# IamJerryXu/Multimodal-Diagnosis-HAM-Spine

Measured on AMD Instinct MI355X. Metric: training images/sec, ResNet50+BERT-base 224px bs32, higher is better.
Workload: dtype bf16; 1 GPU; C2: ResNet50 + BERT-base(L=128) + cross-attention FusionModule + MLP head, 224x224, batch 32 per GPU, CE(label_smoothing=0.02), fused AdamW, train-mode BatchNorm and dropout; per_gpu_batch=32, global_batch=32, seq_len=128, params=134897991, parallelism=dp1

## Files before the change

include/hamspine.h:

```cpp
#ifndef HAMSPINE_H
#define HAMSPINE_H

#include <stdint.h>

#ifdef __cplusplus
extern "C" {
#endif

typedef int hs_status;
enum { HS_OK = 0, HS_ERR_ARG = 1, HS_ERR_HIP = 2, HS_ERR_UNSUPPORTED = 3 };
enum { HS_F32 = 0, HS_BF16 = 1 };

const char* hs_last_error(void);
int hs_version(void);
int hs_device_ok(void);


enum {
    HS_A_KC = 0,
    HS_A_RC = 1,
    HS_A_CONV = 2,
    HS_A_DGRAD = 3
};
enum {
// ... 519 lines not shown
    float* dword;
    float* dpos;
    float* dtype0;
    float* dgamma;
    float* dbeta;
    int32_t n_layers;
    hs_bert_layer_desc layers[HS_BERT_MAX_LAYERS];
    int32_t pack_rows;
} hs_bert_desc;
int32_t hs_bert_pack_rows_available(void);
hs_status hs_bert_query(const hs_bert_desc* d, int64_t* saved_bytes, int64_t* ws_bytes, int64_t* out_offset);
hs_status hs_bert_fwd(const hs_bert_desc* d, const int64_t* ids, const int64_t* mask, void* saved, int64_t saved_bytes,
                      void* ws, int64_t ws_bytes, void* stream);
hs_status hs_bert_bwd(const hs_bert_desc* d, const int64_t* ids, const int64_t* mask, const void* dy, void* saved,
                      int64_t saved_bytes, void* ws, int64_t ws_bytes, void* stream);

hs_status hs_linear_fwd(int32_t dtype, const void* x, int64_t M, int32_t ldx, const hs_linear* lin, const void* w_lp,
                        void* y, int32_t ldy, int32_t out_dtype, int32_t act, void* preact, const void* residual,
                        int32_t ldr, float dropout_p, uint64_t seed, void* stream);
hs_status hs_linear_bwd(int32_t dtype, const void* x, int64_t M, int32_t ldx, const hs_linear* lin, const void* w_lp,
                        const void* dy, int32_t ldy, void* dx, int32_t lddx, int32_t dx_dtype, int32_t mul_mode,
                        const void* mul_src, int32_t ldm, const void* dx_residual, void* ws, int64_t ws_bytes,
                        void* stream);
int64_t hs_linear_bwd_ws_bytes(int64_t M, int32_t in_f, int32_t out_f, int32_t dtype);

hs_status hs_tta_expand(const float* x, float* out, int64_t planes, int32_t H, int32_t W, const int32_t* ops, int32_t V,
                        void* stream);
hs_status hs_group_mean(const float* x, float* out, int32_t V, int64_t n, void* stream);
hs_status hs_repeat(int32_t elem_bytes, const void* x, void* out, int64_t n, int32_t V, void* stream);
hs_status hs_gradcam(int32_t dtype, const void* act, const void* grad, float* cam, int32_t B, int32_t C, int32_t HW,
// ... 35 lines not shown
```

multimodal-diagnosis-ham-spine_amd/hamspine/csrc/blocks.hip:

```cpp
#include <algorithm>
#include <atomic>
#include <mutex>
#include <unordered_map>
#include <vector>
#include "hs_internal.h"
#include "hs_switch.h"
#include "pw_stream.h"

namespace hs {

__global__ __launch_bounds__(256) void gather3_kernel(const float* __restrict__ a, const float* __restrict__ b,
                                                      const float* __restrict__ c, float* __restrict__ dst, int n) {
    const int i = blockIdx.x * 256 + threadIdx.x;
    if (i >= 3 * n) return;
    const int w = i / n, k = i - w * n;
    dst[i] = w == 0 ? a[k] : (w == 1 ? b[k] : c[k]);
}

static inline long long align_up(long long v, long long a) { return (v + a - 1) / a * a; }
static inline int esize(int dt) { return dt == HS_BF16 ? 2 : 4; }

struct Arena {
    char* base = nullptr;
    long long cap = 0, off = 0, peak = 0;
// ... 22 lines not shown
        saved.base = (char*)saved_base; saved.cap = saved_bytes;
        ws.base = (char*)ws_base; ws.cap = ws_bytes;
    }
    hipStream_t side = nullptr;
    bool side_used = false;
    bool defer_wgrad = false;
    GemmGroup *grp_pw = nullptr, *grp_conv = nullptr;
    bool group_nt = false;
    GemmGroup* grp_nt = nullptr;
    GemmGroup* tower_grp = nullptr;
    struct PendTr { const void* src; void* dst; int R, C; long long ld; unsigned char tok; };
    std::vector<PendTr> pend_tr;
    const int *pk_T = nullptr, *pk_cu = nullptr, *pk_row = nullptr, *pk_inv = nullptr;
    const int *pk_kc = nullptr, *pk_kcpos = nullptr, *pk_kcols = nullptr;
    bool kc_on = false;
};

static hipStream_t g_side_stream[16] = {};
static hipEvent_t g_events[16][64] = {};
static int g_event_next[16] = {};
static std::mutex g_side_mu;
static int side_setup(Run& r) {
    if (r.plan || !sw::overlap()) return HS_OK;
    int dev = 0;
    HS_CHECK_HIP(hipGetDevice(&dev));
    if (dev < 0 || dev >= 16) return HS_OK;
    std::lock_guard<std::mutex> lk(g_side_mu);
    if (!g_side_stream[dev]) HS_CHECK_HIP(hipStreamCreateWithFlags(&g_side_stream[dev], hipStreamNonBlocking));
    r.side = g_side_stream[dev];
    return HS_OK;
// ... 1242 lines not shown
    HS_PROPAGATE(linear_fwd_run(r, x, M, Hd, qkv_lin, L.wqkv, L.qkv, 3 * Hd, r.dt, HS_ACT_NONE, nullptr, nullptr, 0, 0.f, 0));
    hs_attn_desc a = bert_attn_desc(d, r.dt);
    const char* qkv = (const char*)L.qkv;
    HS_PROPAGATE(attention_fwd_run(r, a, qkv, qkv ? qkv + (long long)Hd * es : nullptr,
                                   qkv ? qkv + 2ll * Hd * es : nullptr, L.ctx));
    HS_PROPAGATE(linear_fwd_run(r, L.ctx, M, Hd, d.ao, L.wao, L.h1, Hd, r.dt, HS_ACT_NONE, nullptr, x, Hd, d.hidden_dropout,
                                d.seed * 8 + 2));
    CALL(r, ln_fwd(r.dt, L.h1, d.ln1.gamma, d.ln1.beta, L.x1, L.mean1, L.rstd1, M, Hd, d.ln_eps, r.s, r.pk_T));
    HS_PROPAGATE(linear_fwd_run(r, L.x1, M, Hd, d.inter_l, L.wi, L.g, I, r.dt, HS_ACT_GELU, L.u, nullptr, 0, 0.f, 0));
    HS_PROPAGATE(linear_fwd_run(r, L.g, M, I, d.out_l, L.wo, L.h2, Hd, r.dt, HS_ACT_NONE, nullptr, L.x1, Hd,
                                d.hidden_dropout, d.seed * 8 + 3));
    CALL(r, ln_fwd(r.dt, L.h2, d.ln2.gamma, d.ln2.beta, y, L.mean2, L.rstd2, M, Hd, d.ln_eps, r.s, r.pk_T));
    RUN_CHECK_ARENAS(r, "bert_layer_fwd");
    return HS_OK;
}
static int bert_layer_bwd_run(Run& r, const hs_bert_layer_desc& d, const void* x, const void* dy, void* dx) {
    BertLayout L;
    HS_PROPAGATE(bert_layout(r, d, L));
    const int Hd = d.hidden, I = d.inter;
    const long long M = (long long)d.B * d.L;
    const int es = esize(r.dt);
    hs_attn_desc a = bert_attn_desc(d, r.dt);
    void* dh2 = r.ws.alloc(M * Hd * es);
    void* dd2 = r.ws.alloc(M * Hd * es);
    void* dh1 = r.ws.alloc(M * Hd * es);
    void* dd1 = r.ws.alloc(M * Hd * es);
    void* du = r.ws.alloc(M * I * es);
    void* dx1 = r.ws.alloc(M * Hd * es);
    void* dctx = r.ws.alloc(M * Hd * es);
    void* dqkv = r.ws.alloc(M * 3 * Hd * es);
// ... 5 lines not shown
    const bool fuse_ln = sw::fused_ln_bwd();
    const void* g2 = d.hidden_dropout > 0.f ? dd2 : dh2;
    hs_linear out_l_w = d.out_l;
    if (fuse_ln) {
        CALL(r, ln_bwd_pre(r.dt, dy, L.h2, d.ln2.gamma, L.mean2, L.rstd2, dh2, d.ln2.dgamma ? d.ln2.dgamma : scratch,
                           d.ln2.dbeta ? d.ln2.dbeta : (scratch ? scratch + Hd : nullptr),
                           d.hidden_dropout > 0.f ? dd2 : nullptr, d.out_l.db, d.hidden_dropout, d.seed * 8 + 3,
                           ln_ws, ln_ws_bytes, M, Hd, r.s, r.pk_inv));
        out_l_w.db = nullptr;
    } else {
        CALLK(r, 128, ln_bwd(r.dt, dy, L.h2, d.ln2.gamma, L.mean2, L.rstd2, dh2, d.ln2.dgamma ? d.ln2.dgamma : scratch,
                             d.ln2.dbeta ? d.ln2.dbeta : (scratch ? scratch + Hd : nullptr), ln_ws, ln_ws_bytes, M, Hd, r.s, r.pk_inv));
        if (d.hidden_dropout > 0.f && r.pk_T) CALL(r, dropout_rows(r.dt, dh2, dd2, M, Hd, d.hidden_dropout, d.seed * 8 + 3, r.pk_T, r.pk_row, r.s));
        else if (d.hidden_dropout > 0.f) CALL(r, hs_dropout(r.dt, dh2, dd2, M * Hd, d.hidden_dropout, d.seed * 8 + 3, r.s));
    }
    const bool nt = r.dt == HS_BF16 && sw::wgrad_nt() && M % 8 == 0 && Hd % 8 == 0 && I % 8 == 0;
    HS_REQUIRE(!r.pk_T || nt, "bert_layer_bwd: packed rows need the transposed-operand weight gradients (bf16, HAMSPINE_WGRAD_NT on)");
    const long long big_tiles = (long long)ceil_div(3 * Hd, 256) * ceil_div(Hd, 128) + (long long)ceil_div(Hd, 256) * ceil_div(Hd, 128) +
                                (long long)ceil_div(I, 256) * ceil_div(Hd, 128) + (long long)ceil_div(Hd, 256) * ceil_div(I, 128);
    const bool grouped = nt && sw::grouped_bert_wgrad() && !sw::overlap() && big_tiles >= 128;
    char* tA = nt ? (char*)r.ws.alloc(M * (long long)std::max(3 * Hd, I) * 2) : nullptr;
    char* tA_ffn2 = grouped ? (char*)r.ws.alloc(M * (long long)Hd * 2) : tA;
    char* tA_ao = grouped ? (char*)r.ws.alloc(M * (long long)Hd * 2) : tA;
    char* tA_qkv = grouped ? (char*)r.ws.alloc(M * 3ll * Hd * 2) : tA;
    r.group_nt = grouped;
    if (grouped && !r.plan) {
        r.grp_nt = r.tower_grp ? r.tower_grp : gemm_group_open(r.s, (long long)(uintptr_t)d.q.w + 16);
        HS_REQUIRE(r.grp_nt != nullptr, "bert_layer_bwd: cannot set up the grouped weight-gradient launch");
    }
    r.kc_on = r.pk_T && r.pk_kcols && grouped && !r.plan && sw::bert_wgrad_chunks() && gemm_group_takes_k_cols();
    const int* const k_cols = r.kc_on ? r.pk_kcols : nullptr;
    char* tX_g = nt ? (char*)r.ws.alloc(M * (long long)I * 2) : nullptr;
    char* tX_x1 = nt ? (char*)r.ws.alloc(M * (long long)Hd * 2) : nullptr;
    char* tX_ctx = nt ? (char*)r.ws.alloc(M * (long long)Hd * 2) : nullptr;
    char* tX_x = nt ? (char*)r.ws.alloc(M * (long long)Hd * 2) : nullptr;
    auto bias_by_colsum = [&](const hs_linear& lin, const void* dy_rm, int ldy) -> int {
        hs_linear only_b = lin;
        only_b.dw = nullptr;
        return linear_wgrad_run(r, nullptr, M, 0, only_b, dy_rm, ldy);
    };
    auto wgrad = [&](const void* x_rm, const void* xT, int in_f, const hs_linear& lin, const void* dy_rm, int ldy, char* tAk) -> int {
        if (!nt || !lin.dw) {
            const bool keep = r.group_nt;
            r.group_nt = false;
            const int st = linear_wgrad_run(r, x_rm, M, in_f, lin, dy_rm, ldy);
            r.group_nt = keep;
            return st;
        }
        HS_PROPAGATE(transpose_run(r, dy_rm, tAk, M, lin.out_f, ldy, true, true));
        const bool fused_b = lin.db && (r.group_nt || hs_gemm_suggest_split(lin.out_f, in_f, (int)M, r.dt) <= 1) && sw::fused_bias_grad();
        HS_PROPAGATE(linear_wgrad_nt_run(r, xT, tAk, M, in_f, lin.out_f, lin.dw, lin.db, 0, nullptr, nullptr, k_cols));
        if (lin.db && !fused_b) HS_PROPAGATE(bias_by_colsum(lin, dy_rm, ldy));
        return HS_OK;
    };
    const bool dnt = r.dt == HS_BF16 && sw::dgrad_nt() && Hd % 8 == 0 && I % 8 == 0;
    char* wo_t = dnt ? (char*)r.ws.alloc((long long)Hd * I * 2) : nullptr;
    char* wi_t = dnt ? (char*)r.ws.alloc((long long)Hd * I * 2) : nullptr;
    char* wqkv_t = dnt ? (char*)r.ws.alloc(3ll * Hd * Hd * 2) : nullptr;
    {
        const void* src[7];
        void* dst[7];
        int32_t R[7], Cc[7];
        int64_t lds[7], ldd[7];
        unsigned char tok[7];
        int n = 0;
        auto add = [&](const void* s_, void* d_, long long rows, int cols, bool tokens = false) {
            src[n] = s_; dst[n] = d_; R[n] = (int32_t)rows; Cc[n] = cols; lds[n] = cols; ldd[n] = rows; tok[n] = tokens ? (r.kc_on ? 2 : 1) : 0;
            ++n;
        };
        if (nt) {
            add(L.g, tX_g, M, I, true);
            add(L.x1, tX_x1, M, Hd, true);
            add(L.ctx, tX_ctx, M, Hd, true);
            add(x, tX_x, M, Hd, true);
// ... 252 lines not shown
    const hs_conv_bn& cb = d.stem.cb;
    if (cb.dw || cb.dgamma || cb.dbeta) {
        r.saved.off = lo.lay_off[0];
        const long long wm = r.ws.mark();
        HS_PROPAGATE(stem_bwd_run(r, d.stem, r.saved.base ? r.saved.base + lo.y_off[0] : nullptr, dy));
        r.ws.release(wm);
    }
    return milestones_flush(r);
}

struct BertTowerLayout {
    long long ssum_off, stats_off;
    long long y_off[HS_BERT_MAX_LAYERS + 1], lay_off[HS_BERT_MAX_LAYERS + 1];
    long long act_bytes;
    long long map_off, out_off;
};
static void bert_pack_pointers(Run& r, const hs_bert_desc& d, const BertTowerLayout& lo) {
    const int* map = (const int*)(r.saved.base + lo.map_off);
    r.pk_T = map;
    r.pk_cu = map + 4;
    r.pk_row = r.pk_cu + (d.B + 1 + 3) / 4 * 4;
    r.pk_inv = r.pk_row + (long long)d.B * d.L;
    r.pk_kc = map + 1;
    r.pk_kcpos = r.pk_inv + (long long)d.B * d.L;
}
static int bert_check(const hs_bert_desc& d) {
    HS_REQUIRE(d.n_layers >= 0 && d.n_layers <= HS_BERT_MAX_LAYERS, "bert: n_layers %d out of range", d.n_layers);
    HS_REQUIRE(d.B > 0 && d.L > 0 && d.hidden > 0 && d.vocab > 0, "bert: bad dims");
    HS_REQUIRE(d.word && d.pos && d.type0 && d.gamma && d.beta, "bert: null embedding parameter");
    for (int i = 0; i < d.n_layers; ++i)
        HS_REQUIRE(d.layers[i].dtype == d.dtype && d.layers[i].B == d.B && d.layers[i].L == d.L && d.layers[i].hidden == d.hidden,
// ... 3 lines not shown
        for (int i = 0; i < d.n_layers; ++i) {
            const hs_bert_layer_desc& l = d.layers[i];
            HS_REQUIRE(l.heads > 0 && d.hidden == 64 * l.heads && l.inter % 8 == 0, "bert: pack_rows needs head dim 64 (layer %d)", i);
            const int wanted = (l.q.dw != nullptr) + (l.k.dw != nullptr) + (l.v.dw != nullptr);
            HS_REQUIRE(wanted == 0 || wanted == 3, "bert: pack_rows needs the q / k / v weight gradients of layer %d all wanted or all frozen", i);
        }
    }
    return HS_OK;
}
static hs_bert_layer_desc bert_layer_of(const hs_bert_desc& d, int i, const int64_t* mask) {
    hs_bert_layer_desc l = d.layers[i];
    l.attention_mask = mask;
    l.seed = d.seed + 16ull * (unsigned)(i + 1);
    return l;
}
static int bert_fwd_run(Run& r, const hs_bert_desc& d, const int64_t* ids, const int64_t* mask, BertTowerLayout& lo) {
    const long long M = (long long)d.B * d.L;
    const int es = esize(d.dtype);
    lo.act_bytes = M * d.hidden * es;
    lo.map_off = lo.out_off = 0;
    char* out_pad = nullptr;
    if (d.pack_rows) {
        HS_REQUIRE(r.plan || mask, "bert_fwd: pack_rows needs an attention mask");
        lo.map_off = r.saved.mark();
        int* map = (int*)r.saved.alloc(bert_row_map_bytes(d.B, d.L));
        lo.out_off = r.saved.mark();
        out_pad = (char*)r.saved.alloc(lo.act_bytes);
        if (!r.plan) {
            RUN_CHECK_ARENAS(r, "bert_fwd(row map)");
            HS_PROPAGATE(bert_row_map(mask, d.B, d.L, map, r.s));
            bert_pack_pointers(r, d, lo);
// ... 7 lines not shown
    char* x = (char*)r.saved.alloc(lo.act_bytes);
    lo.lay_off[0] = r.saved.mark();
    CALL(r, bert_embed_fwd_rows(d.dtype, ids, d.word, d.pos, d.type0, d.gamma, d.beta, ssum, x, stats, stats + M, M, d.L, d.hidden,
                                d.vocab, d.ln_eps, d.embed_dropout, d.seed, r.pk_T, r.pk_row, r.s));
    for (int i = 0; i < d.n_layers; ++i) {
        lo.y_off[i + 1] = r.saved.mark();
        char* y = (char*)r.saved.alloc(lo.act_bytes);
        lo.lay_off[i + 1] = r.saved.mark();
        const hs_bert_layer_desc l = bert_layer_of(d, i, mask);
        const long long wm = r.ws.mark();
        HS_PROPAGATE(bert_layer_fwd_run(r, l, x, y));
        r.ws.release(wm);
        x = y;
    }
    if (d.pack_rows) CALL(r, bert_unpack_rows(x, out_pad, M, (long long)d.hidden * es, r.pk_inv, r.s));
    return HS_OK;
}
static int bert_bwd_run(Run& r, const hs_bert_desc& d, const int64_t* ids, const int64_t* mask, const void* dy_in,
                        const BertTowerLayout& lo) {
    const long long M = (long long)d.B * d.L;
    const int Hd = d.hidden;
    char* dy_packed = d.pack_rows ? (char*)r.ws.alloc(lo.act_bytes) : nullptr;
    int* kcols = d.pack_rows ? (int*)r.ws.alloc(sizeof(int)) : nullptr;
    char* gbuf[2] = {(char*)r.ws.alloc(lo.act_bytes), (char*)r.ws.alloc(lo.act_bytes)};
    int cur = 0;
    const void* dy = dy_in;
    char* base = r.saved.base;
    if (d.pack_rows && !r.plan) {
        RUN_CHECK_ARENAS(r, "bert_bwd(row map)");
        bert_pack_pointers(r, d, lo);
        HS_PROPAGATE(bert_pack_rows(dy_in, dy_packed, M, (long long)Hd * esize(d.dtype), r.pk_T, r.pk_row, r.pk_kc + 1, kcols, r.s));
        r.pk_kcols = kcols;
        dy = dy_packed;
    }
// ... 1 lines not shown
    int pending = 0;
    long long wm = 0;
    const void* gps[8][16];
    struct HookGuard {
        explicit HookGuard(Run* rr) { gemm_group_set_immediate_hook([](void* c) -> int { return pending_transposes_flush(*(Run*)c); }, rr); }
        ~HookGuard() { gemm_group_set_immediate_hook(nullptr, nullptr); }
    } hook_guard(&r);
    for (int i = d.n_layers - 1; i >= 0; --i) {
        const hs_bert_layer_desc l = bert_layer_of(d, i, mask);
        char* dx = gbuf[cur];
        r.saved.off = lo.lay_off[i + 1];
        if (pending == 0) {
            wm = r.ws.mark();
            r.tower_grp = (span > 1 && !r.plan) ? gemm_group_open(r.s, (long long)(uintptr_t)l.q.w + 24) : nullptr;
        }
        HS_PROPAGATE(bert_layer_bwd_run(r, l, base ? base + lo.y_off[i] : nullptr, dy, dx));
        {
            const void* gp[16] = {l.q.dw, l.q.db, l.k.dw, l.k.db, l.v.dw, l.v.db, l.ao.dw, l.ao.db, l.ln1.dgamma, l.ln1.dbeta,
                                  l.inter_l.dw, l.inter_l.db, l.out_l.dw, l.out_l.db, l.ln2.dgamma, l.ln2.dbeta};
            memcpy(gps[pending], gp, sizeof(gp));
        }
        ++pending;
        if (pending == span || i == 0) {
            HS_PROPAGATE(pending_transposes_flush(r));
            if (r.tower_grp) HS_PROPAGATE(gemm_group_flush(r.tower_grp, r.s));
            r.tower_grp = nullptr;
            r.ws.release(wm);
            for (int k = 0; k < pending; ++k) HS_PROPAGATE(milestones_hit(r, gps[k], 16));
            pending = 0;
        }
        dy = dx;
// ... 389 lines not shown
    for (int i = 0; i < d->n_blocks; ++i) {
        Run q(d->stem.dtype, fake, 1ll << 50, fake, 1ll << 50, nullptr);
        q.saved.off = lo.lay_off[i + 1];
        ResLayout L;
        if (res_layout(q, d->blocks[i], L) != HS_OK) return -1;
        for (int j = 0; j + 1 < d->blocks[i].n_main; ++j) put((char*)L.main[j].a - fake);
        put(lo.y_off[i + 1]);
    }
    return n <= max_entries ? n : -1;
}

hs_status hs_bert_query(const hs_bert_desc* d, int64_t* saved_bytes, int64_t* ws_bytes, int64_t* out_offset) {
    HS_REQUIRE(d, "bert_query: null desc");
    HS_PROPAGATE(bert_check(*d));
    BertTowerLayout lo;
    HS_PROPAGATE(query_fwd_bwd(d->dtype, *d, [&](Run& r) { return bert_fwd_run(r, *d, nullptr, nullptr, lo); },
                               [&](Run& r, const hs_bert_desc& dd) { return bert_bwd_run(r, dd, nullptr, nullptr, nullptr, lo); },
                               saved_bytes, ws_bytes, true));
    if (out_offset) *out_offset = d->pack_rows ? lo.out_off : lo.y_off[d->n_layers];
    return HS_OK;
}
hs_status hs_bert_fwd(const hs_bert_desc* d, const int64_t* ids, const int64_t* mask, void* saved, int64_t saved_bytes,
                      void* ws, int64_t ws_bytes, void* stream) {
    HS_REQUIRE(d && ids && saved && ws, "bert_fwd: null argument");
    HS_PROPAGATE(bert_check(*d));
    BertTowerLayout lo;
    return run_entry("bert_fwd", d->dtype, saved, saved_bytes, ws, ws_bytes, stream, [&](Run& r) {
        return r.plan ? bert_fwd_run(r, *d, nullptr, nullptr, lo) : bert_fwd_run(r, *d, ids, mask, lo);
    });
}
hs_status hs_bert_bwd(const hs_bert_desc* d, const int64_t* ids, const int64_t* mask, const void* dy, void* saved,
                      int64_t saved_bytes, void* ws, int64_t ws_bytes, void* stream) {
    HS_REQUIRE(d && ids && dy && saved && ws, "bert_bwd: null argument");
    HS_PROPAGATE(bert_check(*d));
    BertTowerLayout lo;
    return run_entry("bert_bwd", d->dtype, saved, saved_bytes, ws, ws_bytes, stream, [&](Run& r) {
        HS_PROPAGATE(plan_fwd_for_bwd(r, [&](Run& f) { return bert_fwd_run(f, *d, nullptr, nullptr, lo); }));
        return r.plan ? bert_bwd_run(r, *d, nullptr, nullptr, nullptr, lo) : bert_bwd_run(r, *d, ids, mask, dy, lo);
    });
}
void hs_set_overlap(int32_t on) { hs::sw::set_overlap(on); }
int32_t hs_bert_pack_rows_available(void) { return (hs::sw::wgrad_nt() && hs::sw::fused_attention()) ? 1 : 0; }
hs_status hs_grad_milestones(int32_t n, const void* const* grad_ptrs, void* const* events) {
    HS_REQUIRE(n >= 0 && n <= kMaxMilestones, "grad_milestones: %d entries (max %d)", n, kMaxMilestones);
    HS_REQUIRE(n == 0 || (grad_ptrs && events), "grad_milestones: null argument");
    g_ms.n = n;
    for (int i = 0; i < n; ++i) {
        HS_REQUIRE(grad_ptrs[i] && events[i], "grad_milestones: null entry %d", i);
        g_ms.ptr[i] = grad_ptrs[i];
        g_ms.ev[i] = (hipEvent_t)events[i];
    }
    return HS_OK;
}
int32_t hs_measure_build(void) {
// ... 10 lines not shown
```

multimodal-diagnosis-ham-spine_amd/hamspine/csrc/hs_switch.h:

```cpp
#pragma once
#include <atomic>
#include <stdlib.h>

namespace hs {
namespace sw {

inline long long off_if_0(const char* e, long long d) { return (e && e[0] == '0') ? 0 : d; }
inline long long on_if_1(const char* e, long long d) { return (e && e[0] == '1') ? 1 : d; }
inline long long int_any(const char* e, long long d) { return e ? atoi(e) : d; }
inline long long int_mask15(const char* e, long long d) { return e ? (atoi(e) & 15) : d; }
inline long long int_1to8(const char* e, long long d) { const long long v = e ? atoi(e) : d; return v >= 1 && v <= 8 ? v : d; }
inline long long int_positive(const char* e, long long d) { const long long v = e ? atoll(e) : 0; return v > 0 ? v : d; }

#define HS_SWITCHES(X) \
   \
  X(p8,                 "HAMSPINE_P8",                  off_if_0,     1,   once,     -, "every GEMM on the generic body, none on the phase-pipelined one") \
  X(p8_wgrad,           "HAMSPINE_P8_WGRAD",            off_if_0,     1,   once,     -, "grouped deep-K weight gradients keep the generic 256x128 tiles") \
  X(conv3,              "HAMSPINE_CONV3",               off_if_0,     1,   once,     -, "3x3 stride-1 convolutions on the generic implicit GEMM, not the halo-patch kernel") \
  X(parity_dgrad,       "HAMSPINE_PARITY_DGRAD",        off_if_0,     1,   once,     -, "stride-2 data gradients keep the natural row order") \
  X(pack_xcd_spread,    "HAMSPINE_PACK_XCD_SPREAD",     off_if_0,     1,   settable, hs_set_pack_xcd_spread, "packed-row launches do not deal their live tiles over all XCDs") \
  X(persistent,         "HAMSPINE_PERSISTENT",          on_if_1,      0,   once,     -, "persistent GEMM launches (measured: no gain)") \
  X(epi_hist,           "HAMSPINE_EPI_HIST",            on_if_1,      0,   once,     -, "measurement: count the epilogue feature sets of the launches, print at exit") \
  X(group_debug,        "HAMSPINE_GROUP_DEBUG",         on_if_1,      0,   once,     -, "measurement: report every upload of a grouped launch's problem table") \
  X(split_units,        "HAMSPINE_SPLIT_UNITS",         int_positive, 512, once,     -, "measurement: the number of workgroups split-K aims at") \
  X(split_max,          "HAMSPINE_SPLIT_MAX",           int_positive, 64,  once,     -, "measurement: the largest split-K factor") \
   \
  X(fused_attention,    "HAMSPINE_FUSED_ATTENTION",     off_if_0,     1,   once,     -, "the unfused attention path") \
   \
  X(overlap,            "HAMSPINE_OVERLAP",             on_if_1,      0,   settable, hs_set_overlap, "a composite's weight gradients run on a side stream beside its data-gradient chain") \
  X(wgrad_nt,           "HAMSPINE_WGRAD_NT",            off_if_0,     1,   settable, hs_set_wgrad_nt, "BertLayer weight gradients from the row-major operands (tn); no packed rows then") \
  X(bert_wgrad_chunks,  "HAMSPINE_BERT_WGRAD_CHUNKS",   off_if_0,     1,   settable, hs_set_bert_wgrad_chunks, "packed text tower: weight gradients walk every padded column") \
  X(grouped_bert_wgrad, "HAMSPINE_GROUPED_BERT_WGRAD",  off_if_0,     1,   once,     -, "every weight-gradient GEMM of a BertLayer on its own") \
  X(wgrad_layers,       "HAMSPINE_WGRAD_LAYERS",        int_1to8,     2,   once,     -, "BERT layers whose weight gradients share one grouped grid (1: flush per layer)") \
  X(dgrad_nt,           "HAMSPINE_DGRAD_NT",            off_if_0,     1,   once,     -, "BERT data gradients read the row-contiguous weights") \
  X(defer_transposes,   "HAMSPINE_DEFER_TRANSPOSES",    off_if_0,     1,   once,     -, "one launch per dY^T where the gradient appears") \
  X(fused_bias_grad,    "HAMSPINE_FUSED_BIAS_GRAD",     off_if_0,     1,   once,     -, "bias gradients by separate column-sum passes") \
  X(fused_ln_bwd,       "HAMSPINE_FUSED_LN_BWD",        off_if_0,     1,   once,     -, "separate LayerNorm-backward / dropout / column-sum passes") \
  X(grouped_wgrad,      "HAMSPINE_GROUPED_WGRAD",       off_if_0,     1,   once,     -, "the image tower backward launches every weight gradient on its own") \
  X(staged_wgrad,       "HAMSPINE_STAGED_WGRAD",        off_if_0,     1,   once,     -, "with gradient milestones, the grouped weight gradients still run only at the end") \
  X(fused_bn_stats,     "HAMSPINE_FUSED_BN_STATS",      off_if_0,     1,   once,     -, "BatchNorm makes its own statistics pass") \
  X(bn_finish,          "HAMSPINE_BN_FINISH",           off_if_0,     1,   once,     -, "BatchNorm finishes its statistics in its own launch") \
  X(fused_bn_bwd,       "HAMSPINE_FUSED_BN_BWD",        off_if_0,     1,   once,     -, "BatchNorm backward makes its own partial-sum pass") \
  X(bnb_finish,         "HAMSPINE_BNB_FINISH",          on_if_1,      0,   once,     -, "the data-gradient GEMM also finishes the BatchNorm-backward sums (measured: no gain)") \
  X(bn_mask_from_x,     "HAMSPINE_BN_MASK_FROM_X",      on_if_1,      0,   once,     -, "inner-stage BatchNorm backward recomputes the ReLU mask from the convolution output (measured neutral)") \
  X(pw_stream,          "HAMSPINE_PW_STREAM",           on_if_1,      0,   once,     -, "1x1 convolutions of a training step through the streaming kernel (measured: a wash)") \
  X(xblock_bn,          "HAMSPINE_XBLOCK_BN",           int_any,      1,   per_call, -, "0: no BatchNorm sums across the block boundary; 2: on every eligible block, whatever its size") \
  X(ds_compact,         "HAMSPINE_DS_COMPACT",          off_if_0,     1,   per_call, -, "bf16 downsample data gradients keep the full-size parity-ordered route") \
  X(img_lean,           "HAMSPINE_IMG_LEAN",            int_mask15,   13,  per_call, -, "bit mask of the bf16 image tower's four lean passes (0: the separate launches)")
#define HS_SWITCHES_MEASURE(X) \
  X(knockout,           "HAMSPINE_KNOCKOUT",            int_any,      0,   once,     -, "bit mask of launch classes left OUT of the step (results are then garbage)")
// ... 28 lines not shown
```

multimodal-diagnosis-ham-spine_amd/hamspine/rt.py:

```python
import ctypes as C
import threading

import torch

from . import _lib as L

_tls = threading.local()
_ws = {}
_seed_lock = threading.Lock()
_seed_state = {"base": None, "ctr": 0}


def stream():
    return C.c_void_p(torch.cuda.current_stream().cuda_stream)


def workspace(nbytes, device):
    key = (device.index if device.index is not None else torch.cuda.current_device(), threading.get_ident(),
           torch.cuda.current_stream().cuda_stream)
    t = _ws.get(key)
    if t is None or t.numel() < nbytes:
        t = torch.empty(max(int(nbytes * 1.25), 1 << 20), dtype=torch.uint8, device=device)
        _ws[key] = t
    return t
# ... 23 lines not shown

def tower_stream(device):
    idx = device.index if device.index is not None else torch.cuda.current_device()
    s = _tower_streams.get(idx)
    if s is None:
        import os
        s = torch.cuda.Stream(device=idx, priority=int(os.environ.get("HAMSPINE_TOWER_PRIORITY", "0")))
        _tower_streams[idx] = s
    return s


def side_streams():
    return list(_tower_streams.values())


def run_on_tower_stream(fn, *inputs):
    cur = torch.cuda.current_stream()
    side = tower_stream(cur.device)
    side.wait_stream(cur)
    for t in inputs:
        if torch.is_tensor(t):
            t.record_stream(side)
    with torch.cuda.stream(side):
        out = fn()

    def join(*outs):
        cur.wait_stream(side)
        for t in outs:
            if torch.is_tensor(t):
                t.record_stream(cur)
    return out, join


_grad_arena = {}
_arena_version = [0]


def grad_arena_register(param, view):
    _grad_arena[param.data_ptr()] = view
    _arena_version[0] += 1


def grad_arena_clear():
    _grad_arena.clear()
    _arena_version[0] += 1
# ... 315 lines not shown
```

multimodal-diagnosis-ham-spine_amd/hamspine/tower.py:

```python
import os
import ctypes as C

import torch
from torch.autograd import Function
from torch.nn.modules import module as _nn_module

import hamspine

from . import _lib as L
from . import rt

_CACHE_ATTR = "_hamspine_tower_cache"
DEBUG_KEEP = None


def _has_hooks(root):
    if (_nn_module._global_forward_hooks or _nn_module._global_forward_pre_hooks or _nn_module._global_backward_hooks or
            getattr(_nn_module, "_global_backward_pre_hooks", None)):
        return True
    key = tuple(map(id, root._modules.values()))
    cached = root.__dict__.get("_hamspine_module_list")
    if cached is None or cached[0] != key:
        cached = (key, list(root.modules()))
        root.__dict__["_hamspine_module_list"] = cached
# ... 352 lines not shown
        if dtype == torch.bfloat16:
            for i in range(len(model.encoder.layer)):
                b = 5 + 16 * i
                self.shadow_groups += [[params[b], params[b + 2], params[b + 4]], [params[b + 6]], [params[b + 10]], [params[b + 12]]]

    def valid_for(self, params):
        if self.arena_version != rt.arena_version():
            return False
        return all(p.data_ptr() == q for p, q in zip(params, self.param_ptrs))


class BertTowerFn(Function):

    @staticmethod
    def forward(ctx, ids, mask, holder, *params):
        model, training, pack_rows = holder
        rt.need_gpu(ids, mask, *params)
        ids = ids.contiguous()
        if ids.dtype != torch.int64:
            ids = ids.long()
        B, Lq = ids.shape
        if Lq > model.embeddings.position_embeddings.weight.shape[0]:
            raise ValueError(f"sequence length {Lq} exceeds max_position_embeddings")
        dtype = hamspine.compute_dtype()
        needs = tuple(ctx.needs_input_grad[3:])
        pack_rows = bool(pack_rows) and bert_pack_supported(model, B, Lq, dtype, mask, needs)
        key = ("bert", B, Lq, dtype, training, needs, pack_rows)
        cache = model.__dict__.setdefault(_CACHE_ATTR, {})
        ent = cache.get(key)
        if ent is None or not ent.valid_for(params):
            ent = cache[key] = _BertEntry(model, B, Lq, dtype, training, params, needs, ids.device, pack_rows)
        rt.ensure_shadows(ent.shadow_groups)
        saved = torch.empty(ent.saved_bytes, dtype=torch.uint8, device=ids.device)
        ws = rt.workspace(ent.ws_bytes, ids.device)
        seed = (rt.next_seed() * 64) & 0xFFFFFFFFFFFFFFFF if training else 0
        ent.desc.seed = seed
        L.check(L.lib().hs_bert_fwd(C.byref(ent.desc), ids.data_ptr(), rt.p(mask), saved.data_ptr(), saved.numel(),
                                    ws.data_ptr(), ws.numel(), rt.stream()), "hs_bert_fwd")
        Bq, Lq2, H = ent.shape
        es = 2 if dtype == torch.bfloat16 else 4
        out = saved[ent.out_off:ent.out_off + Bq * Lq2 * H * es].view(dtype).view(Bq, Lq2, H)
        ctx.ent, ctx.saved_buf, ctx.seed = ent, saved, seed
        ctx.ids, ctx.mask, ctx.params = ids, mask, params
        ctx.counted = _forward_begins(ent, needs)
        ctx.save_for_backward(out)
        return out

    @staticmethod
    def backward(ctx, dy):
        ent, saved, params = ctx.ent, ctx.saved_buf, ctx.params
        if saved is None:
            raise RuntimeError("hamspine.tower: backward through a tower a second time: its saved activations are freed by the "
                               "first backward (retain_graph=True is not supported on the tower nodes)")
        _ = ctx.saved_tensors
        rt.wgrad_defer_flush_all()
        dy = dy.contiguous()
        if dy.dtype != ent.dtype:
            dy = dy.to(ent.dtype)
        desc, views = ent.desc, ent.make_views
        if _shared_buffer_unsafe(ent, params):
# ... 2 lines not shown
        ws = rt.workspace(ent.ws_bytes, saved.device)

        def call():
            L.check(L.lib().hs_bert_bwd(C.byref(desc), ctx.ids.data_ptr(), rt.p(ctx.mask), dy.data_ptr(), saved.data_ptr(),
                                        saved.numel(), ws.data_ptr(), ws.numel(), rt.stream()), "hs_bert_bwd")
        if desc is ent.desc:
            _with_milestones(ent, params, call)
        else:
            call()
        ctx.saved_buf = None
        if ctx.counted is not None:
            ctx.counted.finish()
        return (None, None, None, *views())


def _bert_desc_with_fresh_grads(ent, params, needs, device):
    store = _GradStore(params, needs, device)
    d = L.BertDesc()
    C.memmove(C.byref(d), C.byref(ent.desc), C.sizeof(L.BertDesc))
    d.dword, d.dpos, d.dtype0, d.dgamma, d.dbeta = (store.ptr(i) for i in range(5))
    gi = 5
    for i in range(d.n_layers):
        ld = d.layers[i]
        g = [store.ptr(gi + k) for k in range(16)]
        ld.q.dw, ld.q.db, ld.k.dw, ld.k.db, ld.v.dw, ld.v.db, ld.ao.dw, ld.ao.db = g[:8]
        ld.ln1.dgamma, ld.ln1.dbeta = g[8], g[9]
        ld.inter_l.dw, ld.inter_l.db, ld.out_l.dw, ld.out_l.db = g[10:14]
        ld.ln2.dgamma, ld.ln2.dbeta = g[14], g[15]
        gi += 16
    return d, store.views
# ... 14 lines not shown
            if any(qkv) and not all(qkv):
                return False
    return all(H == 64 * layer._heads and layer._inter % 8 == 0 for layer in model.encoder.layer)


def bert_ran_packed(hidden):
    ent = getattr(getattr(hidden, "grad_fn", None), "ent", None)
    return getattr(ent, "pack_rows", None)


def bert_hidden(model, input_ids, attention_mask, skip_padded_rows=False):
    if not (towers_enabled() and input_ids.is_cuda and input_ids.dim() == 2):
        return None
    if _has_hooks(model):
        return None
    return BertTowerFn.apply(input_ids, attention_mask, (model, model.training, bool(skip_padded_rows)), *bert_params(model))
```

Baseline: 3311 images/s.

## Precompute BERT backward transposes after forward on the tower side stream

Adds an hs_bert_bwd_prepare entry that, right after the BERT forward, transposes the gradient-independent activations and weights each layer's backward needs into extra space reserved in the saved buffer. It is launched on the tower side stream after the join, so it can overlap with the image tower and fusion work. The backward then looks up a prep record keyed by the saved buffer and skips its own transpose launch per layer. The cost is a larger saved buffer (more memory), a global prep table, and a fallback path when the record does not match.

```diff
diff --git a/include/hamspine.h b/include/hamspine.h
--- a/include/hamspine.h
+++ b/include/hamspine.h
@@ -557,6 +557,9 @@
                       void* ws, int64_t ws_bytes, void* stream);
 hs_status hs_bert_bwd(const hs_bert_desc* d, const int64_t* ids, const int64_t* mask, const void* dy, void* saved,
                       int64_t saved_bytes, void* ws, int64_t ws_bytes, void* stream);
+hs_status hs_bert_bwd_prepare(const hs_bert_desc* d, const int64_t* ids, const int64_t* mask, void* saved, int64_t saved_bytes,
+                              void* ws, int64_t ws_bytes, void* stream);
+void hs_bert_prepare_counters(int64_t* out);
 
 hs_status hs_linear_fwd(int32_t dtype, const void* x, int64_t M, int32_t ldx, const hs_linear* lin, const void* w_lp,
                         void* y, int32_t ldy, int32_t out_dtype, int32_t act, void* preact, const void* residual,
diff --git a/multimodal-diagnosis-ham-spine_amd/hamspine/csrc/blocks.hip b/multimodal-diagnosis-ham-spine_amd/hamspine/csrc/blocks.hip
--- a/multimodal-diagnosis-ham-spine_amd/hamspine/csrc/blocks.hip
+++ b/multimodal-diagnosis-ham-spine_amd/hamspine/csrc/blocks.hip
@@ -4,6 +4,7 @@
 #include <unordered_map>
 #include <vector>
 #include "hs_internal.h"
+#include "hs_prep_table.h"
 #include "hs_switch.h"
 #include "pw_stream.h"
 
@@ -60,6 +61,7 @@
     const int *pk_T = nullptr, *pk_cu = nullptr, *pk_row = nullptr, *pk_inv = nullptr;
     const int *pk_kc = nullptr, *pk_kcpos = nullptr, *pk_kcols = nullptr;
     bool kc_on = false;
+    const PrepLayer* prep = nullptr;
 };
 
 static hipStream_t g_side_stream[16] = {};
@@ -1332,6 +1334,40 @@
     RUN_CHECK_ARENAS(r, "bert_layer_fwd");
     return HS_OK;
 }
+struct BertBwdMode {
+    bool nt, dnt, grouped, kc;
+    unsigned char bits() const { return (unsigned char)(1 | (nt ? 2 : 0) | (dnt ? 4 : 0) | (grouped ? 8 : 0) | (kc ? 16 : 0)); }
+};
+static BertBwdMode bert_bwd_mode(int dt, const hs_bert_layer_desc& d, bool packed) {
+    const int Hd = d.hidden, I = d.inter;
+    const long long M = (long long)d.B * d.L;
+    BertBwdMode m;
+    m.nt = dt == HS_BF16 && sw::wgrad_nt() && M % 8 == 0 && Hd % 8 == 0 && I % 8 == 0;
+    const long long big_tiles = (long long)ceil_div(3 * Hd, 256) * ceil_div(Hd, 128) + (long long)ceil_div(Hd, 256) * ceil_div(Hd, 128) +
+                                (long long)ceil_div(I, 256) * ceil_div(Hd, 128) + (long long)ceil_div(Hd, 256) * ceil_div(I, 128);
+    m.grouped = m.nt && sw::grouped_bert_wgrad() && !sw::overlap() && big_tiles >= 128;
+    m.dnt = dt == HS_BF16 && sw::dgrad_nt() && Hd % 8 == 0 && I % 8 == 0;
+    m.kc = packed && m.grouped && sw::bert_wgrad_chunks() && gemm_group_takes_k_cols();
+    return m;
+}
+static void bert_prep_alloc(Arena& a, const hs_bert_layer_desc& d, void* p[PREP_OPERANDS]) {
+    const int Hd = d.hidden, I = d.inter;
+    const long long M = (long long)d.B * d.L;
+    p[PREP_TX_G] = a.alloc(M * (long long)I * 2);
+    p[PREP_TX_X1] = a.alloc(M * (long long)Hd * 2);
+    p[PREP_TX_CTX] = a.alloc(M * (long long)Hd * 2);
+    p[PREP_TX_X] = a.alloc(M * (long long)Hd * 2);
+    p[PREP_WO_T] = a.alloc((long long)Hd * I * 2);
+    p[PREP_WI_T] = a.alloc((long long)Hd * I * 2);
+    p[PREP_WQKV_T] = a.alloc(3ll * Hd * Hd * 2);
+}
+static bool bert_prep_wanted(int dt, const hs_bert_layer_desc& d, bool packed) {
+    if (!sw::bert_prep() || dt != HS_BF16) return false;
+    const BertBwdMode m = bert_bwd_mode(dt, d, packed);
+    return m.nt && m.dnt && (d.q.dw || d.k.dw || d.v.dw || d.ao.dw || d.inter_l.dw || d.out_l.dw);
+}
+static std::atomic<long long> g_prep_launch_calls{0}, g_prep_entries{0}, g_prep_layers_used{0}, g_prep_layers_self{0};
+
 static int bert_layer_bwd_run(Run& r, const hs_bert_layer_desc& d, const void* x, const void* dy, void* dx) {
     BertLayout L;
     HS_PROPAGATE(bert_layout(r, d, L));
@@ -1367,11 +1403,10 @@
         if (d.hidden_dropout > 0.f && r.pk_T) CALL(r, dropout_rows(r.dt, dh2, dd2, M, Hd, d.hidden_dropout, d.seed * 8 + 3, r.pk_T, r.pk_row, r.s));
         else if (d.hidden_dropout > 0.f) CALL(r, hs_dropout(r.dt, dh2, dd2, M * Hd, d.hidden_dropout, d.seed * 8 + 3, r.s));
     }
-    const bool nt = r.dt == HS_BF16 && sw::wgrad_nt() && M % 8 == 0 && Hd % 8 == 0 && I % 8 == 0;
+    const BertBwdMode mode = bert_bwd_mode(r.dt, d, r.pk_T != nullptr);
+    const bool nt = mode.nt;
     HS_REQUIRE(!r.pk_T || nt, "bert_layer_bwd: packed rows need the transposed-operand weight gradients (bf16, HAMSPINE_WGRAD_NT on)");
-    const long long big_tiles = (long long)ceil_div(3 * Hd, 256) * ceil_div(Hd, 128) + (long long)ceil_div(Hd, 256) * ceil_div(Hd, 128) +
-                                (long long)ceil_div(I, 256) * ceil_div(Hd, 128) + (long long)ceil_div(Hd, 256) * ceil_div(I, 128);
-    const bool grouped = nt && sw::grouped_bert_wgrad() && !sw::overlap() && big_tiles >= 128;
+    const bool grouped = mode.grouped;
     char* tA = nt ? (char*)r.ws.alloc(M * (long long)std::max(3 * Hd, I) * 2) : nullptr;
     char* tA_ffn2 = grouped ? (char*)r.ws.alloc(M * (long long)Hd * 2) : tA;
     char* tA_ao = grouped ? (char*)r.ws.alloc(M * (long long)Hd * 2) : tA;
@@ -1381,7 +1416,9 @@
         r.grp_nt = r.tower_grp ? r.tower_grp : gemm_group_open(r.s, (long long)(uintptr_t)d.q.w + 16);
         HS_REQUIRE(r.grp_nt != nullptr, "bert_layer_bwd: cannot set up the grouped weight-gradient launch");
     }
-    r.kc_on = r.pk_T && r.pk_kcols && grouped && !r.plan && sw::bert_wgrad_chunks() && gemm_group_takes_k_cols();
+    const PrepLayer* const pre = (!r.plan && r.prep && r.prep->made && r.prep->mode == mode.bits()) ? r.prep : nullptr;
+    r.kc_on = pre ? (pre->mode & 16) != 0 && r.pk_kcols : (mode.kc && r.pk_kcols && !r.plan);
+    if (pre && grouped && r.grp_nt) gemm_group_upload_on_stream(r.grp_nt);
     const int* const k_cols = r.kc_on ? r.pk_kcols : nullptr;
     char* tX_g = nt ? (char*)r.ws.alloc(M * (long long)I * 2) : nullptr;
     char* tX_x1 = nt ? (char*)r.ws.alloc(M * (long long)Hd * 2) : nullptr;
@@ -1406,11 +1443,16 @@
         if (lin.db && !fused_b) HS_PROPAGATE(bias_by_colsum(lin, dy_rm, ldy));
         return HS_OK;
     };
-    const bool dnt = r.dt == HS_BF16 && sw::dgrad_nt() && Hd % 8 == 0 && I % 8 == 0;
+    const bool dnt = mode.dnt;
     char* wo_t = dnt ? (char*)r.ws.alloc((long long)Hd * I * 2) : nullptr;
     char* wi_t = dnt ? (char*)r.ws.alloc((long long)Hd * I * 2) : nullptr;
     char* wqkv_t = dnt ? (char*)r.ws.alloc(3ll * Hd * Hd * 2) : nullptr;
-    {
+    if (pre) {
+        tX_g = (char*)pre->p[PREP_TX_G]; tX_x1 = (char*)pre->p[PREP_TX_X1]; tX_ctx = (char*)pre->p[PREP_TX_CTX]; tX_x = (char*)pre->p[PREP_TX_X];
+        wo_t = (char*)pre->p[PREP_WO_T]; wi_t = (char*)pre->p[PREP_WI_T]; wqkv_t = (char*)pre->p[PREP_WQKV_T];
+        g_prep_layers_used.fetch_add(1, std::memory_order_relaxed);
+    } else {
+        if (!r.plan) g_prep_layers_self.fetch_add(1, std::memory_order_relaxed);
         const void* src[7];
         void* dst[7];
         int32_t R[7], Cc[7];
@@ -1693,7 +1735,10 @@
     long long y_off[HS_BERT_MAX_LAYERS + 1], lay_off[HS_BERT_MAX_LAYERS + 1];
     long long act_bytes;
     long long map_off, out_off;
+    long long prep_off[HS_BERT_MAX_LAYERS];
+    long long base_bytes;
 };
+static_assert(kPrepMaxLayers == HS_BERT_MAX_LAYERS, "hs_prep_table.h: kPrepMaxLayers");
 static void bert_pack_pointers(Run& r, const hs_bert_desc& d, const BertTowerLayout& lo) {
     const int* map = (const int*)(r.saved.base + lo.map_off);
     r.pk_T = map;
@@ -1727,7 +1772,7 @@
     l.seed = d.seed + 16ull * (unsigned)(i + 1);
     return l;
 }
-static int bert_fwd_run(Run& r, const hs_bert_desc& d, const int64_t* ids, const int64_t* mask, BertTowerLayout& lo) {
+static int bert_fwd_run(Run& r, const hs_bert_desc& d, const int64_t* ids, const int64_t* mask, BertTowerLayout& lo, bool reserve_prep) {
     const long long M = (long long)d.B * d.L;
     const int es = esize(d.dtype);
     lo.act_bytes = M * d.hidden * es;
@@ -1765,10 +1810,64 @@
         x = y;
     }
     if (d.pack_rows) CALL(r, bert_unpack_rows(x, out_pad, M, (long long)d.hidden * es, r.pk_inv, r.s));
+    lo.base_bytes = r.saved.mark();
+    for (int i = 0; i < d.n_layers; ++i) {
+        lo.prep_off[i] = -1;
+        if (!reserve_prep || !bert_prep_wanted(d.dtype, d.layers[i], d.pack_rows != 0)) continue;
+        lo.prep_off[i] = r.saved.mark();
+        void* p[PREP_OPERANDS];
+        bert_prep_alloc(r.saved, d.layers[i], p);
+    }
+    return HS_OK;
+}
+static PrepTable g_prep;
+static int bert_prepare_run(Run& r, const hs_bert_desc& d, const BertTowerLayout& lo, PrepRecord& rec) {
+    if (r.plan) return HS_OK;
+    if (d.pack_rows) bert_pack_pointers(r, d, lo);
+    std::vector<const void*> src;
+    std::vector<void*> dst;
+    std::vector<int32_t> R, Cc;
+    std::vector<int64_t> lds, ldd;
+    std::vector<unsigned char> tok;
+    auto add = [&](const void* s_, void* d_, long long rows, int cols, unsigned char t) {
+        src.push_back(s_); dst.push_back(d_); R.push_back((int32_t)rows); Cc.push_back(cols); lds.push_back(cols); ldd.push_back(rows);
+        tok.push_back(t);
+    };
+    char* base = r.saved.base;
+    for (int i = 0; i < d.n_layers; ++i) {
+        if (lo.prep_off[i] < 0) continue;
+        const hs_bert_layer_desc l = bert_layer_of(d, i, nullptr);
+        const int Hd = l.hidden, I = l.inter;
+        const long long M = (long long)l.B * l.L;
+        const BertBwdMode mode = bert_bwd_mode(d.dtype, l, d.pack_rows != 0);
+        BertLayout L;
+        r.saved.off = lo.lay_off[i + 1];
+        HS_PROPAGATE(bert_layout(r, l, L));
+        PrepLayer& pl = rec.layer[i];
+        r.saved.off = lo.prep_off[i];
+        bert_prep_alloc(r.saved, l, pl.p);
+        RUN_CHECK_ARENAS(r, "bert_bwd_prepare");
+        pl.made = true;
+        pl.mode = mode.bits();
+        const unsigned char t = d.pack_rows ? (mode.kc ? 2 : 1) : 0;
+        add(L.g, pl.p[PREP_TX_G], M, I, t);
+        add(L.x1, pl.p[PREP_TX_X1], M, Hd, t);
+        add(L.ctx, pl.p[PREP_TX_CTX], M, Hd, t);
+        add(base + lo.y_off[i], pl.p[PREP_TX_X], M, Hd, t);
+        add(L.wo, pl.p[PREP_WO_T], Hd, I, 0);
+        add(L.wi, pl.p[PREP_WI_T], I, Hd, 0);
+        add(L.wqkv, pl.p[PREP_WQKV_T], 3 * Hd, Hd, 0);
+    }
+    const int n = (int)src.size();
+    if (n == 0) return HS_OK;
+    CALLK(r, 4, transpose_bf16_multi_rows(n, src.data(), dst.data(), R.data(), Cc.data(), lds.data(), ldd.data(), r.pk_inv, tok.data(), r.pk_kc,
+                                          r.pk_kcpos, r.s));
+    g_prep_launch_calls.fetch_add(ceil_div(n, HS_TRANSPOSE_MAX), std::memory_order_relaxed);
+    g_prep_entries.fetch_add(n, std::memory_order_relaxed);
     return HS_OK;
 }
 static int bert_bwd_run(Run& r, const hs_bert_desc& d, const int64_t* ids, const int64_t* mask, const void* dy_in,
-                        const BertTowerLayout& lo) {
+                        const BertTowerLayout& lo, const PrepRecord* prep = nullptr) {
     const long long M = (long long)d.B * d.L;
     const int Hd = d.hidden;
     char* dy_packed = d.pack_rows ? (char*)r.ws.alloc(lo.act_bytes) : nullptr;
@@ -1800,7 +1899,10 @@
             wm = r.ws.mark();
             r.tower_grp = (span > 1 && !r.plan) ? gemm_group_open(r.s, (long long)(uintptr_t)l.q.w + 24) : nullptr;
         }
-        HS_PROPAGATE(bert_layer_bwd_run(r, l, base ? base + lo.y_off[i] : nullptr, dy, dx));
+        r.prep = (prep && !r.plan) ? &prep->layer[i] : nullptr;
+        const int st_layer = bert_layer_bwd_run(r, l, base ? base + lo.y_off[i] : nullptr, dy, dx);
+        r.prep = nullptr;
+        HS_PROPAGATE(st_layer);
         {
             const void* gp[16] = {l.q.dw, l.q.db, l.k.dw, l.k.db, l.v.dw, l.v.db, l.ao.dw, l.ao.db, l.ln1.dgamma, l.ln1.dbeta,
                                   l.inter_l.dw, l.inter_l.db, l.out_l.dw, l.out_l.db, l.ln2.dgamma, l.ln2.dbeta};
@@ -2220,7 +2322,7 @@
     HS_REQUIRE(d, "bert_query: null desc");
     HS_PROPAGATE(bert_check(*d));
     BertTowerLayout lo;
-    HS_PROPAGATE(query_fwd_bwd(d->dtype, *d, [&](Run& r) { return bert_fwd_run(r, *d, nullptr, nullptr, lo); },
+    HS_PROPAGATE(query_fwd_bwd(d->dtype, *d, [&](Run& r) { return bert_fwd_run(r, *d, nullptr, nullptr, lo, true); },
                                [&](Run& r, const hs_bert_desc& dd) { return bert_bwd_run(r, dd, nullptr, nullptr, nullptr, lo); },
                                saved_bytes, ws_bytes, true));
     if (out_offset) *out_offset = d->pack_rows ? lo.out_off : lo.y_off[d->n_layers];
@@ -2231,19 +2333,64 @@
     HS_REQUIRE(d && ids && saved && ws, "bert_fwd: null argument");
     HS_PROPAGATE(bert_check(*d));
     BertTowerLayout lo;
+    g_prep.erase(saved);
+    bool room = d->dtype == HS_BF16 && sw::bert_prep();
+    if (room) {
+        Run pl(d->dtype);
+        HS_PROPAGATE(bert_fwd_run(pl, *d, nullptr, nullptr, lo, true));
+        room = pl.saved.peak <= saved_bytes;
+    }
     return run_entry("bert_fwd", d->dtype, saved, saved_bytes, ws, ws_bytes, stream, [&](Run& r) {
-        return r.plan ? bert_fwd_run(r, *d, nullptr, nullptr, lo) : bert_fwd_run(r, *d, ids, mask, lo);
+        return r.plan ? bert_fwd_run(r, *d, nullptr, nullptr, lo, room) : bert_fwd_run(r, *d, ids, mask, lo, room);
     });
+}
+hs_status hs_bert_bwd_prepare(const hs_bert_desc* d, const int64_t* ids, const int64_t* mask, void* saved, int64_t saved_bytes,
+                              void* ws, int64_t ws_bytes, void* stream) {
+    HS_REQUIRE(d && ids && saved && ws, "bert_bwd_prepare: null argument");
+    (void)mask;
+    HS_PROPAGATE(bert_check(*d));
+    BertTowerLayout lo;
+    PrepRecord rec;
+    g_prep.erase(saved);
+    HS_PROPAGATE(run_entry("bert_bwd_prepare", d->dtype, saved, saved_bytes, ws, ws_bytes, stream, [&](Run& r) {
+        HS_PROPAGATE(plan_fwd_for_bwd(r, [&](Run& f) { return bert_fwd_run(f, *d, nullptr, nullptr, lo, true); }));
+        return bert_prepare_run(r, *d, lo, rec);
+    }));
+    bool any = false;
+    for (int i = 0; i < d->n_layers; ++i) any = any || rec.layer[i].made;
+    if (!any) return HS_OK;
+    rec.saved_bytes = saved_bytes;
+    rec.stream = stream;
+    rec.B = d->B; rec.L = d->L; rec.hidden = d->hidden; rec.n_layers = d->n_layers; rec.pack_rows = d->pack_rows;
+    rec.span = (int)sw::wgrad_layers();
+    rec.overlap = (int)sw::overlap();
+    g_prep.insert(saved, rec);
+    return HS_OK;
+}
+static bool bert_prep_usable(const PrepRecord& rec, const hs_bert_desc& d, long long saved_bytes, void* stream) {
+    return rec.saved_bytes == saved_bytes && rec.stream == stream && rec.B == d.B && rec.L == d.L && rec.hidden == d.hidden &&
+           rec.n_layers == d.n_layers && rec.pack_rows == d.pack_rows && rec.span == (int)sw::wgrad_layers() &&
+           rec.overlap == (int)sw::overlap();
 }
 hs_status hs_bert_bwd(const hs_bert_desc* d, const int64_t* ids, const int64_t* mask, const void* dy, void* saved,
                       int64_t saved_bytes, void* ws, int64_t ws_bytes, void* stream) {
     HS_REQUIRE(d && ids && dy && saved && ws, "bert_bwd: null argument");
     HS_PROPAGATE(bert_check(*d));
     BertTowerLayout lo;
+    PrepRecord rec;
+    const bool prepared = g_prep.take(saved, &rec) && bert_prep_usable(rec, *d, saved_bytes, stream);
     return run_entry("bert_bwd", d->dtype, saved, saved_bytes, ws, ws_bytes, stream, [&](Run& r) {
-        HS_PROPAGATE(plan_fwd_for_bwd(r, [&](Run& f) { return bert_fwd_run(f, *d, nullptr, nullptr, lo); }));
-        return r.plan ? bert_bwd_run(r, *d, nullptr, nullptr, nullptr, lo) : bert_bwd_run(r, *d, ids, mask, dy, lo);
+        HS_PROPAGATE(plan_fwd_for_bwd(r, [&](Run& f) { return bert_fwd_run(f, *d, nullptr, nullptr, lo, false); }));
+        return r.plan ? bert_bwd_run(r, *d, nullptr, nullptr, nullptr, lo) : bert_bwd_run(r, *d, ids, mask, dy, lo, prepared ? &rec : nullptr);
     });
+}
+void hs_bert_prepare_counters(int64_t* out) {
+    if (!out) return;
+    out[0] = g_prep_launch_calls.load(std::memory_order_relaxed);
+    out[1] = g_prep_entries.load(std::memory_order_relaxed);
+    out[2] = g_prep_layers_used.load(std::memory_order_relaxed);
+    out[3] = g_prep_layers_self.load(std::memory_order_relaxed);
+    out[4] = (int64_t)g_prep.size();
 }
 void hs_set_overlap(int32_t on) { hs::sw::set_overlap(on); }
 int32_t hs_bert_pack_rows_available(void) { return (hs::sw::wgrad_nt() && hs::sw::fused_attention()) ? 1 : 0; }
diff --git a/multimodal-diagnosis-ham-spine_amd/hamspine/csrc/hs_prep_table.h b/multimodal-diagnosis-ham-spine_amd/hamspine/csrc/hs_prep_table.h
--- /dev/null
+++ b/multimodal-diagnosis-ham-spine_amd/hamspine/csrc/hs_prep_table.h
@@ -0,0 +1,53 @@
+#pragma once
+#include <mutex>
+#include <unordered_map>
+
+namespace hs {
+
+constexpr int kPrepMaxLayers = 24;
+enum { PREP_TX_G = 0, PREP_TX_X1, PREP_TX_CTX, PREP_TX_X, PREP_WO_T, PREP_WI_T, PREP_WQKV_T, PREP_OPERANDS };
+
+struct PrepLayer {
+    bool made = false;
+    unsigned char mode = 0;
+    void* p[PREP_OPERANDS] = {};
+};
+struct PrepRecord {
+    long long saved_bytes = 0;
+    void* stream = nullptr;
+    int B = 0, L = 0, hidden = 0, n_layers = 0, pack_rows = 0;
+    int span = 0, overlap = 0;
+    PrepLayer layer[kPrepMaxLayers];
+};
+
+class PrepTable {
+public:
+    static constexpr size_t kMaxRecords = 64;
+    void erase(const void* key) {
+        std::lock_guard<std::mutex> lk(mu_);
+        map_.erase(key);
+    }
+    void insert(const void* key, const PrepRecord& rec) {
+        std::lock_guard<std::mutex> lk(mu_);
+        if (map_.size() >= kMaxRecords && map_.find(key) == map_.end()) map_.clear();
+        map_[key] = rec;
+    }
+    bool take(const void* key, PrepRecord* out) {
+        std::lock_guard<std::mutex> lk(mu_);
+        auto it = map_.find(key);
+        if (it == map_.end()) return false;
+        *out = it->second;
+        map_.erase(it);
+        return true;
+    }
+    size_t size() {
+        std::lock_guard<std::mutex> lk(mu_);
+        return map_.size();
+    }
+
+private:
+    std::mutex mu_;
+    std::unordered_map<const void*, PrepRecord> map_;
+};
+
+}
diff --git a/multimodal-diagnosis-ham-spine_amd/hamspine/csrc/hs_switch.h b/multimodal-diagnosis-ham-spine_amd/hamspine/csrc/hs_switch.h
--- a/multimodal-diagnosis-ham-spine_amd/hamspine/csrc/hs_switch.h
+++ b/multimodal-diagnosis-ham-spine_amd/hamspine/csrc/hs_switch.h
@@ -33,7 +33,8 @@
   X(grouped_bert_wgrad, "HAMSPINE_GROUPED_BERT_WGRAD",  off_if_0,     1,   once,     -, "every weight-gradient GEMM of a BertLayer on its own") \
   X(wgrad_layers,       "HAMSPINE_WGRAD_LAYERS",        int_1to8,     2,   once,     -, "BERT layers whose weight gradients share one grouped grid (1: flush per layer)") \
   X(dgrad_nt,           "HAMSPINE_DGRAD_NT",            off_if_0,     1,   once,     -, "BERT data gradients read the row-contiguous weights") \
-  X(defer_transposes,   "HAMSPINE_DEFER_TRANSPOSES",    off_if_0,     1,   once,     -, "one launch per dY^T where the gradient appears") \
+  X(bert_prep,          "HAMSPINE_BERT_PREP",           off_if_0,     1,   per_call, -, "the text tower's backward makes its gradient-independent transposes itself; no room for them in `saved`") \
+  X(defer_transposes,   "HAMSPINE_DEFER_TRANSPOSES",   off_if_0,     1,   once,     -, "one launch per dY^T where the gradient appears") \
   X(fused_bias_grad,    "HAMSPINE_FUSED_BIAS_GRAD",     off_if_0,     1,   once,     -, "bias gradients by separate column-sum passes") \
   X(fused_ln_bwd,       "HAMSPINE_FUSED_LN_BWD",        off_if_0,     1,   once,     -, "separate LayerNorm-backward / dropout / column-sum passes") \
   X(grouped_wgrad,      "HAMSPINE_GROUPED_WGRAD",       off_if_0,     1,   once,     -, "the image tower backward launches every weight gradient on its own") \
diff --git a/multimodal-diagnosis-ham-spine_amd/hamspine/rt.py b/multimodal-diagnosis-ham-spine_amd/hamspine/rt.py
--- a/multimodal-diagnosis-ham-spine_amd/hamspine/rt.py
+++ b/multimodal-diagnosis-ham-spine_amd/hamspine/rt.py
@@ -61,6 +61,17 @@
     return list(_tower_streams.values())
 
 
+_after_join = threading.local()
+
+
+def after_tower_join(call):
+    calls = getattr(_after_join, "calls", None)
+    if calls is None:
+        return False
+    calls.append(call)
+    return True
+
+
 def run_on_tower_stream(fn, *inputs):
     cur = torch.cuda.current_stream()
     side = tower_stream(cur.device)
@@ -68,14 +79,26 @@
     for t in inputs:
         if torch.is_tensor(t):
             t.record_stream(side)
-    with torch.cuda.stream(side):
-        out = fn()
+    calls = []
+    outer = getattr(_after_join, "calls", None)
+    _after_join.calls = calls
+    try:
+        with torch.cuda.stream(side):
+            out = fn()
+    finally:
+        _after_join.calls = outer
 
     def join(*outs):
         cur.wait_stream(side)
         for t in outs:
             if torch.is_tensor(t):
                 t.record_stream(cur)
+        if calls:
+            todo = calls[:]
+            del calls[:]
+            with torch.cuda.stream(side):
+                for c in todo:
+                    c()
     return out, join
 
 
diff --git a/multimodal-diagnosis-ham-spine_amd/hamspine/tower.py b/multimodal-diagnosis-ham-spine_amd/hamspine/tower.py
--- a/multimodal-diagnosis-ham-spine_amd/hamspine/tower.py
+++ b/multimodal-diagnosis-ham-spine_amd/hamspine/tower.py
@@ -390,7 +390,8 @@
 
     @staticmethod
     def forward(ctx, ids, mask, holder, *params):
-        model, training, pack_rows = holder
+        model, training, pack_rows = holder[:3]
+        will_backprop = holder[3] if len(holder) > 3 else True
         rt.need_gpu(ids, mask, *params)
         ids = ids.contiguous()
         if ids.dtype != torch.int64:
@@ -401,7 +402,9 @@
         dtype = hamspine.compute_dtype()
         needs = tuple(ctx.needs_input_grad[3:])
         pack_rows = bool(pack_rows) and bert_pack_supported(model, B, Lq, dtype, mask, needs)
-        key = ("bert", B, Lq, dtype, training, needs, pack_rows)
+        prep = will_backprop and bert_prepare_enabled() and dtype == torch.bfloat16 and any(needs[5 + 16 * i + k] for i in range(len(model.encoder.layer))
+                                                                          for k in _BERT_WEIGHT_SLOTS)
+        key = ("bert", B, Lq, dtype, training, needs, pack_rows, prep)
         cache = model.__dict__.setdefault(_CACHE_ATTR, {})
         ent = cache.get(key)
         if ent is None or not ent.valid_for(params):
@@ -420,6 +423,14 @@
         ctx.ids, ctx.mask, ctx.params = ids, mask, params
         ctx.counted = _forward_begins(ent, needs)
         ctx.save_for_backward(out)
+        if prep:
+            desc, mask_p = ent.desc, rt.p(mask)
+
+            def prepare():
+                L.check(L.lib().hs_bert_bwd_prepare(C.byref(desc), ids.data_ptr(), mask_p, saved.data_ptr(), saved.numel(),
+                                                    ws.data_ptr(), ws.numel(), rt.stream()), "hs_bert_bwd_prepare")
+            if not rt.after_tower_join(prepare):
+                prepare()
         return out
 
     @staticmethod
@@ -452,6 +463,13 @@
         return (None, None, None, *views())
 
 
+_BERT_WEIGHT_SLOTS = (0, 2, 4, 6, 10, 12)
+
+
+def bert_prepare_enabled():
+    return os.environ.get("HAMSPINE_BERT_PREP", "1") != "0"
+
+
 def _bert_desc_with_fresh_grads(ent, params, needs, device):
     store = _GradStore(params, needs, device)
     d = L.BertDesc()
@@ -496,4 +514,5 @@
         return None
     if _has_hooks(model):
         return None
-    return BertTowerFn.apply(input_ids, attention_mask, (model, model.training, bool(skip_padded_rows)), *bert_params(model))
+    return BertTowerFn.apply(input_ids, attention_mask, (model, model.training, bool(skip_padded_rows), torch.is_grad_enabled()),
+                             *bert_params(model))
```

Measured after the change: 3123 images/s. 0.943x the previous value.
